# superxslam/SuperOdom

Hardware: AMD Instinct MI355X
Metric: icp_registrations_per_sec (higher is better)
Workload: dtype f64

## Files before the change

superodom_amd/csrc/kernels.hip:

```cpp
#include <hip/hip_runtime.h>
#include <hip/hip_ext.h>

#include <cstddef>
#include <cstdlib>
#include <cstring>
#include <type_traits>

#ifdef SO_LM_STAMPS
#define SO_LM_STAMP(dbg, i) do { if (dbg) (dbg)[i] = wall_clock64(); } while (0)
#endif
#include "kernels.h"
#include "plane_fit.h"

namespace soicp {

#define SO_MATCH_SUCCESS 0
#define SO_MATCH_NOT_ENOUGH 1
#define SO_MATCH_TOO_FAR 2
#define SO_MATCH_BAD_PCA 3
#define SO_MATCH_INVALID 4
#define SO_MATCH_MSE 5
#define SO_MATCH_DROPPED 254
#define SO_MATCH_PENDING 255
static_assert(SO_FIT_SUCCESS == SO_MATCH_SUCCESS && SO_FIT_BAD_PCA == SO_MATCH_BAD_PCA && SO_FIT_INVALID == SO_MATCH_INVALID && SO_FIT_MSE == SO_MATCH_MSE,
// ... 1423 lines not shown
            for (int step = 8; step >= 1; step >>= 1) r = (r + step < 16 && rowoff[r + step] <= t) ? r + step : r;
            cn[u] = rowbeg[r] + (t - rowoff[r]);
            const float4 p = mpts[cn[u]];
            ax_[u] = p.x; ay_[u] = p.y; az_[u] = p.z;
          }
        }
#pragma unroll
        for (int u = 0; u < 4; ++u)
          if (cn[u] != 0xFFFFFFFFu) loc.insert(((unsigned long long)__float_as_uint(l2_d2(qx, qy, qz, ax_[u], ay_[u], az_[u])) << 32) | cn[u]);
      }
      unsigned long long m5[5];
#pragma unroll
      for (int t = 0; t < 5; ++t) {
        m5[t] = wave_min_u64(loc.b0);
        if (loc.b0 == m5[t] && m5[t] != ~0ull) { loc.b0 = loc.b1; loc.b1 = loc.b2; loc.b2 = loc.b3; loc.b3 = loc.b4; loc.b4 = ~0ull; }
      }
      if (lane == 0) {
        const float d2_4 = __uint_as_float((uint32_t)(m5[4] >> 32));
        int stq = SO_MATCH_PENDING;
        if (m5[4] == ~0ull || (double)d2_4 > (double)mp.sq_max_dist_f) stq = SO_MATCH_TOO_FAR;
        else {
          uint32_t* o = nbr5 + (size_t)5 * i;
          __builtin_nontemporal_store((uint32_t)m5[0], o); __builtin_nontemporal_store((uint32_t)m5[1], o + 1);
          __builtin_nontemporal_store((uint32_t)m5[2], o + 2); __builtin_nontemporal_store((uint32_t)m5[3], o + 3);
          __builtin_nontemporal_store((uint32_t)m5[4], o + 4);
        }
        __builtin_nontemporal_store((uint8_t)stq, &status[i]);
      }
    }
  }
}

constexpr int kNAcc = 29;

__device__ __forceinline__ uint32_t query_of(uint32_t vb, uint32_t V, int tid, uint32_t q) { return vb * 256u + (uint32_t)tid + q * V * 256u; }

__device__ __forceinline__ bool eval_slot_active(const DevState* st, int slot) {
  return !st->reg_done && (slot == 0 || st->lm_more);
}

struct LmCtl {
  double T[7];
  int32_t lm_max, outer_iter, max_outer, pad;
};

__device__ __forceinline__ int lm_solve_finished(DevState* st, const LmCtl& ctl, const double x[7], double count, int lm_iterations,
                                                 int num_successful, int termination, double initial_cost, double x_cost, const LmSums& sums) {
  for (int i = 0; i < 7; ++i) st->T[i] = x[i];
  const int o = ctl.outer_iter;
  DevIterStats& is = st->iters[o < 16 ? o : 15];
  relative_motion(ctl.T, x, is.translation_norm, is.rotation_norm);
  is.num_surf = (int32_t)count; is.lm_iterations = lm_iterations; is.num_successful = num_successful;
  is.termination = termination; is.initial_cost = initial_cost; is.final_cost = x_cost;
  for (int h = 0; h < 7; ++h) is.reject_hist[h] = (int32_t)sums.hist[h];
  for (int h = 0; h < 9; ++h) is.obs_hist[h] = (int32_t)sums.hist[7 + h];
  for (int i = 0; i < 7; ++i) is.pose_after[i] = x[i];
  st->outer_iter = o + 1;
  st->n_iterations = o + 1;
  if (num_successful == 1 || o + 1 >= ctl.max_outer) {
    st->reg_done = 1;
    for (int i = 0; i < 7; ++i) st->T_final[i] = x[i];
    st->done_count = st->done_count + 1u;
    return 1;
  }
  return 0;
}

__device__ __forceinline__ int lm_control_regs(int slot, DevState* st, LmState& S, const LmSums& sums, const LmCtl& ctl, bool persist,
                                               int* reg_done_out = nullptr) {
  if (reg_done_out) *reg_done_out = 0;
  int more;
  double unused_pose[7];
  double* next_pose = persist ? unused_pose : st->eval_pose;
  if (slot == 0) more = lm_begin(S, ctl.T, sums, ctl.lm_max, next_pose);
#ifdef SO_LM_STAMPS
  else more = lm_feed(S, sums, next_pose, slot == 1 ? st->dbg : nullptr);
#else
  else more = lm_feed(S, sums, next_pose);
#endif
  if (!persist || !more) st->lm_more = more;
  if (more) return 1;
  const int rd = lm_solve_finished(st, ctl, S.x, S.count, S.lm_iterations, S.num_successful, S.termination, S.initial_cost, S.x_cost, sums);
  if (rd) {
    if (reg_done_out) *reg_done_out = 1;
    const bool have = S.count > 0;
    for (int i = 0; i < 36; ++i) st->JtJ[i] = have ? S.H[i] : 0.0;
    for (int i = 0; i < 6; ++i) st->Jtr[i] = have ? S.g[i] : 0.0;
  }
  return 0;
}

typedef unsigned int u4v __attribute__((ext_vector_type(4)));
__device__ __forceinline__ void store16_sc1(u4v* p, u4v v) { asm volatile("global_store_dwordx4 %0, %1, off sc1" ::"v"(p), "v"(v) : "memory"); }
__device__ __forceinline__ u4v load16_sc1(const u4v* p) {
  u4v v;
  asm volatile("global_load_dwordx4 %0, %1, off sc1\n\ts_waitcnt vmcnt(0)" : "=v"(v) : "v"(p) : "memory");
  return v;
}

__device__ __forceinline__ void store16_sys(u4v* p, u4v v) { asm volatile("global_store_dwordx4 %0, %1, off sc0 sc1" ::"v"(p), "v"(v) : "memory"); }
__device__ __forceinline__ u4v load16_sys(const u4v* p) {
  u4v v;
  asm volatile("global_load_dwordx4 %0, %1, off sc0 sc1\n\ts_waitcnt vmcnt(0)" : "=v"(v) : "v"(p) : "memory");
  return v;
}

#define SO_LM_INLINE __forceinline__
__device__ SO_LM_INLINE int lm_control(int slot, DevState* st, LmState& S_lds, const LmSums& sums_lds, const LmCtl& ctl, bool persist = false,
                                       u4v* hand = nullptr, unsigned long long want = 0, double* pose_out = nullptr, int* reg_done_out = nullptr) {
  LmState S;
#pragma unroll
  for (int i = 0; i < 7; ++i) { S.x[i] = S_lds.x[i]; S.cand[i] = S_lds.cand[i]; }
#pragma unroll
  for (int i = 0; i < 6; ++i) {
    S.g[i] = S_lds.g[i]; S.scale[i] = S_lds.scale[i]; S.diag[i] = S_lds.diag[i];
#pragma unroll
    for (int j = i; j < 6; ++j) { S.H[6 * i + j] = S_lds.H[6 * i + j]; S.H[6 * j + i] = S.H[6 * i + j]; }
  }
  S.x_cost = S_lds.x_cost; S.x_norm = S_lds.x_norm; S.inv_radius = S_lds.inv_radius; S.decrease_factor = S_lds.decrease_factor;
  S.inv_model_cost_change = S_lds.inv_model_cost_change; S.step_norm = S_lds.step_norm; S.cand_norm = S_lds.cand_norm;
  S.model_cost_change = S_lds.model_cost_change; S.initial_cost = S_lds.initial_cost; S.count = S_lds.count;
  S.iter = S_lds.iter; S.max_iter = S_lds.max_iter; S.reuse_diagonal = S_lds.reuse_diagonal; S.invalid_steps = S_lds.invalid_steps;
  S.num_successful = S_lds.num_successful; S.termination = S_lds.termination; S.done = S_lds.done; S.lm_iterations = S_lds.lm_iterations;
  const int more_ = lm_control_regs(slot, st, S, sums_lds, ctl, persist, reg_done_out);
  if (hand) {
#pragma unroll
    for (int k = 0; k < 8; ++k) {
      const unsigned long long val = (k < 7) ? (unsigned long long)__double_as_longlong(S.cand[k < 7 ? k : 0]) : (unsigned long long)more_;
      const u4v v = {(unsigned int)val, (unsigned int)(val >> 32), (unsigned int)want, (unsigned int)(want >> 32)};
      store16_sc1(hand + k, v);
    }
#pragma unroll
    for (int k = 0; k < 7; ++k) pose_out[k] = S.cand[k];
  }
#pragma unroll
  for (int i = 0; i < 7; ++i) { S_lds.x[i] = S.x[i]; S_lds.cand[i] = S.cand[i]; }
#pragma unroll
  for (int i = 0; i < 6; ++i) {
    S_lds.g[i] = S.g[i]; S_lds.scale[i] = S.scale[i]; S_lds.diag[i] = S.diag[i];
#pragma unroll
    for (int j = i; j < 6; ++j) { S_lds.H[6 * i + j] = S.H[6 * i + j]; S_lds.H[6 * j + i] = S.H[6 * i + j]; }
  }
  S_lds.x_cost = S.x_cost; S_lds.x_norm = S.x_norm; S_lds.inv_radius = S.inv_radius; S_lds.decrease_factor = S.decrease_factor;
  S_lds.inv_model_cost_change = S.inv_model_cost_change; S_lds.step_norm = S.step_norm; S_lds.cand_norm = S.cand_norm;
  S_lds.model_cost_change = S.model_cost_change; S_lds.initial_cost = S.initial_cost; S_lds.count = S.count;
  S_lds.iter = S.iter; S_lds.max_iter = S.max_iter; S_lds.reuse_diagonal = S.reuse_diagonal; S_lds.invalid_steps = S.invalid_steps;
  S_lds.num_successful = S.num_successful; S_lds.termination = S.termination; S_lds.done = S.done; S_lds.lm_iterations = S.lm_iterations;
#ifdef SO_LM_STAMPS
  if (slot == 1) st->dbg[7] = wall_clock64();
#endif
  return more_;
}

__device__ __forceinline__ int lm_control_wave(int slot, DevState* st, LmState& S, const LmSums& sums, const LmCtl& ctl, double* gather ,
                                               u4v* hand, unsigned long long want, double* pose_out, int* reg_done_out, int lane,
                                               unsigned long long* dbg = nullptr) {
  const bool is_mat = lane < 36, is_vec = lane >= 36 && lane < 42;
  const int li = is_mat ? lane / 6 : 0, lj = is_mat ? lane - 6 * li : (is_vec ? lane - 36 : 0);
  const int la = li < lj ? li : lj, lb = li < lj ? lj : li;
  const int tri = 6 * la - (la * (la - 1)) / 2 + (lb - la);
  const bool is_diag = is_mat && li == lj;
  double x[7], cand[7];
  double x_cost, x_norm, inv_radius, decrease_factor, mcc_state, initial_cost, count, inv_mcc, step_norm, cand_norm;
  int iter, max_iter, reuse_diagonal, invalid_steps, num_successful, termination, done, lm_iterations;
  double Hl = 0, gl = 0, diag_l = 0, sa = 1.0, sb = 1.0;
  int more = 0;
  bool propose = false;
  if (slot == 0) {
#pragma unroll
    for (int i = 0; i < 7; ++i) { x[i] = ctl.T[i]; cand[i] = x[i]; }
    iter = 0; max_iter = ctl.lm_max; reuse_diagonal = 0; invalid_steps = 0; num_successful = 0; termination = 0; done = 0; lm_iterations = 0;
    inv_radius = LmConst::kInitialInvRadius; decrease_factor = 2.0; mcc_state = 0; inv_mcc = 0; step_norm = 0; cand_norm = 0;
    count = sums.count; x_cost = sums.cost; initial_cost = x_cost; x_norm = 0;
    if (is_mat) Hl = sums.JtJ[tri];
    if (is_vec) gl = sums.Jtr[lj];
    if (!(count > 0)) { termination = 4; done = 1; }
    else {
      const double sc = 1.0 / (1.0 + sqrt(Hl));
      if (is_diag) S.scale[li] = sc;
      __builtin_amdgcn_fence(__ATOMIC_ACQ_REL, "wavefront");
      sa = S.scale[is_vec ? lj : la]; sb = S.scale[lb];
      double n2 = 0;
#pragma unroll
      for (int i = 0; i < 7; ++i) n2 = SO_FMA(x[i], x[i], n2);
      x_norm = sqrt(n2);
      propose = true;
    }
  } else {
#pragma unroll
    for (int i = 0; i < 7; ++i) { x[i] = S.x[i]; cand[i] = S.cand[i]; }
    x_cost = S.x_cost; x_norm = S.x_norm; inv_radius = S.inv_radius; decrease_factor = S.decrease_factor; mcc_state = S.model_cost_change;
    initial_cost = S.initial_cost; count = S.count; inv_mcc = S.inv_model_cost_change; step_norm = S.step_norm; cand_norm = S.cand_norm;
    iter = S.iter; max_iter = S.max_iter; reuse_diagonal = S.reuse_diagonal; invalid_steps = S.invalid_steps; num_successful = S.num_successful;
    termination = S.termination; done = S.done; lm_iterations = S.lm_iterations;
    if (is_mat) { Hl = S.H[lane]; sa = S.scale[la]; sb = S.scale[lb]; }
    if (is_vec) { gl = S.g[lj]; sa = S.scale[lj]; }
    if (is_diag) diag_l = S.diag[li];
    if (!done) {
      SO_LM_STAMP(dbg, 0);
      const double cand_cost = sums.cost;
      if (step_norm <= LmConst::kParameterTolerance * (x_norm + LmConst::kParameterTolerance)) { termination = 2; done = 1; }
      else {
        const double cost_change = x_cost - cand_cost;
        if (fabs(cost_change) <= LmConst::kFunctionTolerance * x_cost) { termination = 1; done = 1; }
        else {
          const double rel = cost_change * inv_mcc;
          SO_LM_STAMP(dbg, 1);
          if (rel > LmConst::kMinRelativeDecrease) {
#pragma unroll
            for (int i = 0; i < 7; ++i) x[i] = cand[i];
            x_norm = cand_norm; x_cost = cand_cost;
            if (is_mat) Hl = sums.JtJ[tri];
            if (is_vec) gl = sums.Jtr[lj];
            num_successful++;
            const double u = 2.0 * rel - 1.0;
            double f = 1.0 - u * u * u;
            if (f < 1.0 / 3.0) f = 1.0 / 3.0;
            inv_radius = inv_radius * f;
            if (inv_radius < LmConst::kMinInvRadius) inv_radius = LmConst::kMinInvRadius;
            decrease_factor = 2.0; reuse_diagonal = 0;
            if (iter >= max_iter) { termination = 0; done = 1; }
            else propose = true;
          } else {
            inv_radius = inv_radius * decrease_factor; decrease_factor *= 2.0; reuse_diagonal = 1;
            propose = true;
          }
          SO_LM_STAMP(dbg, 2);
        }
      }
    }
  }
  if (propose && reuse_diagonal == 0) {
    const double xi = lane == 36 ? x[0] : (lane == 37 ? x[1] : x[2]);
    const bool big = lane >= 36 && lane < 39 && fabs(gl) > 1e-6 && fabs(xi) < 1e5;
    if (__ballot(big) == 0ull) {
      if (is_vec) gather[48 + lj] = gl;
      __builtin_amdgcn_fence(__ATOMIC_ACQ_REL, "wavefront");
      double gu[6];
#pragma unroll
      for (int i = 0; i < 6; ++i) gu[i] = gather[48 + i];
      if (lm_gradient_max_norm(x, gu) <= LmConst::kGradientTolerance) { termination = 3; done = 1; propose = false; }
    }
  }
  double scale_u[6];
#pragma unroll
  for (int i = 0; i < 6; ++i) scale_u[i] = 1.0;
  if (propose) {
#pragma unroll
    for (int i = 0; i < 6; ++i) scale_u[i] = S.scale[i];
  }
  while (propose) {
    if (iter >= max_iter) { termination = 0; done = 1; break; }
    if (inv_radius >= LmConst::kMaxInvRadius) { termination = 5; done = 1; break; }
    iter++; lm_iterations = iter;
    if (!reuse_diagonal) {
      double v = Hl * sa * sa;
      v = v < LmConst::kMinLmDiagonal ? LmConst::kMinLmDiagonal : v;
      diag_l = v > LmConst::kMaxLmDiagonal ? LmConst::kMaxLmDiagonal : v;
    }
    const double Hs = Hl * sa * sb;
    const double damp = diag_l * inv_radius;
    const double Al = is_diag ? Hs + damp : Hs;
    if (is_mat) gather[lane] = Al;
    if (is_diag) gather[42 + li] = Hs;
    if (is_vec) gather[36 + lj] = gl * sa;
    __builtin_amdgcn_fence(__ATOMIC_ACQ_REL, "wavefront");
    double A[36], gs[6], y[6], step[6];
#pragma unroll
    for (int i = 0; i < 6; ++i) {
#pragma unroll
      for (int j = 0; j <= i; ++j) A[6 * i + j] = gather[6 * i + j];
      gs[i] = gather[36 + i];
    }
    SO_LM_STAMP(dbg, 3);
    const bool ok = lm_chol6(A, gs, y);
    SO_LM_STAMP(dbg, 4);
    reuse_diagonal = 1;
    double mcc = 0;
    if (ok) {
      double sHs = 0, sg = 0;
#pragma unroll
      for (int i = 0; i < 6; ++i) { step[i] = -y[i]; sg = SO_FMA(step[i], gs[i], sg); }
#pragma unroll
      for (int i = 0; i < 6; ++i) {
        double r = 0;
#pragma unroll
        for (int j = i + 1; j < 6; ++j) r = SO_FMA(gather[6 * i + j], step[j], r);
        sHs = SO_FMA(step[i], SO_FMA(gather[42 + i], step[i], 2.0 * r), sHs);
      }
      mcc = SO_FMA(-0.5, sHs, -sg);
    }
    __builtin_amdgcn_fence(__ATOMIC_ACQ_REL, "wavefront");
    if (!ok || !(mcc > 0.0)) {
      if (++invalid_steps >= LmConst::kMaxConsecutiveInvalidSteps) { termination = 5; done = 1; break; }
      inv_radius *= 2.0;
      continue;
    }
    SO_LM_STAMP(dbg, 5);
    invalid_steps = 0;
    mcc_state = mcc;
    double delta[6];
#pragma unroll
    for (int i = 0; i < 6; ++i) delta[i] = step[i] * scale_u[i];
    pose_plus(x, delta, cand);
    SO_LM_STAMP(dbg, 6);
    more = 1;
    break;
  }
  {
    double hv = cand[0];
    hv = lane == 1 ? cand[1] : hv; hv = lane == 2 ? cand[2] : hv; hv = lane == 3 ? cand[3] : hv;
    hv = lane == 4 ? cand[4] : hv; hv = lane == 5 ? cand[5] : hv; hv = lane == 6 ? cand[6] : hv;
    const unsigned long long val = lane == 7 ? (unsigned long long)more : (unsigned long long)__double_as_longlong(hv);
    if (lane < 8) {
      const u4v v = {(unsigned int)val, (unsigned int)(val >> 32), (unsigned int)want, (unsigned int)(want >> 32)};
      store16_sc1(hand + lane, v);
    }
    if (lane < 7) pose_out[lane] = hv;
  }
  if (more) {
    inv_mcc = 1.0 / mcc_state;
    double sn = 0, n2 = 0;
#pragma unroll
    for (int i = 0; i < 7; ++i) sn = SO_FMA(x[i] - cand[i], x[i] - cand[i], sn);
#pragma unroll
    for (int i = 0; i < 7; ++i) n2 = SO_FMA(cand[i], cand[i], n2);
    step_norm = sqrt(sn); cand_norm = sqrt(n2);
  }
  if (is_mat) S.H[lane] = Hl;
  if (is_vec) S.g[lj] = gl;
  if (is_diag) S.diag[li] = diag_l;
  if (slot == 0 && termination == 4 && lane < 6) S.scale[lane] = 1.0;
  if (lane == 0) {
#pragma unroll
    for (int i = 0; i < 7; ++i) { S.x[i] = x[i]; S.cand[i] = cand[i]; }
    S.x_cost = x_cost; S.x_norm = x_norm; S.inv_radius = inv_radius; S.decrease_factor = decrease_factor; S.model_cost_change = mcc_state;
    S.initial_cost = initial_cost; S.count = count; S.inv_model_cost_change = inv_mcc; S.step_norm = step_norm; S.cand_norm = cand_norm;
    S.iter = iter; S.max_iter = max_iter; S.reuse_diagonal = reuse_diagonal; S.invalid_steps = invalid_steps; S.num_successful = num_successful;
    S.termination = termination; S.done = done; S.lm_iterations = lm_iterations;
  }
#ifdef SO_LM_STAMPS
  if (slot == 1 && lane == 0) st->dbg[7] = wall_clock64();
#endif
  if (!more) {
    int rd = 0;
    if (lane == 0) {
      st->lm_more = 0;
      rd = lm_solve_finished(st, ctl, x, count, lm_iterations, num_successful, termination, initial_cost, x_cost, sums);
      *reg_done_out = rd;
    }
    rd = __builtin_amdgcn_readfirstlane(rd);
    if (rd) {
      const bool have = count > 0;
      if (is_mat) st->JtJ[lane] = have ? Hl : 0.0;
      if (is_vec) st->Jtr[lj] = have ? gl : 0.0;
    }
  } else if (lane == 0) *reg_done_out = 0;
  return more;
}

__device__ __forceinline__ void load_ctl(LmCtl& ctl, const DevState* st, int tid, int first) {
  const int k = tid - first;
  if (k >= 0 && k < 7) ctl.T[k] = st->T[k];
  else if (k == 7) ctl.lm_max = st->lm_max;
  else if (k == 8) ctl.outer_iter = st->outer_iter;
  else if (k == 9) ctl.max_outer = st->max_outer;
}

__device__ __forceinline__ void publish_state(const DevState* st, const EvalParams& ep, int outer, int tid, int nthreads) {
  publish_state_to(ep.hring[outer & 1], st, ep.seq_base | (unsigned long long)(outer + 1), tid, nthreads);
}
__device__ __forceinline__ void publish_state_to(DevState* dst, const DevState* st, unsigned long long seq, int tid, int nthreads) {
  if (!dst) return;
  __threadfence_block();
  __syncthreads();
  const unsigned long long* src = reinterpret_cast<const unsigned long long*>(st);
  unsigned long long* out = reinterpret_cast<unsigned long long*>(dst);
  constexpr int kWords = (int)(offsetof(DevState, seq) / 8);
  for (int i = tid; i < kWords; i += nthreads) out[i] = src[i];
  __threadfence_system();
  __syncthreads();
  if (tid == 0) __hip_atomic_store(&dst->seq, seq, __ATOMIC_RELEASE, __HIP_MEMORY_SCOPE_SYSTEM);
}

__device__ __forceinline__ void copy_words(double* dst, const double* src, int n_doubles, int tid, int nthreads) {
  for (int i = tid; i < n_doubles; i += nthreads) dst[i] = src[i];
}
static_assert(sizeof(LmState) % 8 == 0 && sizeof(LmSums) % 8 == 0, "controller state must be double-aligned");

constexpr int kPartStride = SO_SOLVE_BLOCKS;
static_assert(kEvalBlocks <= kPartStride && kFitBlocksMax <= kPartStride && kNAcc <= kSumsStride, "partials table");
constexpr int kRedStride = kNAcc + 2;

template <int CTRL>
__device__ __forceinline__ double dpp_f64(double v) {
  const int lo = __builtin_amdgcn_update_dpp(0, __double2loint(v), CTRL, 0xF, 0xF, false);
  const int hi = __builtin_amdgcn_update_dpp(0, __double2hiint(v), CTRL, 0xF, 0xF, false);
  return __hiloint2double(hi, lo);
}
__device__ __forceinline__ double swap32_add(double a, double b) {
  const auto lo = __builtin_amdgcn_permlane32_swap((unsigned)__double2loint(a), (unsigned)__double2loint(b), false, false);
  const auto hi = __builtin_amdgcn_permlane32_swap((unsigned)__double2hiint(a), (unsigned)__double2hiint(b), false, false);
  return __hiloint2double((int)hi[0], (int)lo[0]) + __hiloint2double((int)hi[1], (int)lo[1]);
}
__device__ __forceinline__ double swap16_add(double a, double b) {
  const auto lo = __builtin_amdgcn_permlane16_swap((unsigned)__double2loint(a), (unsigned)__double2loint(b), false, false);
  const auto hi = __builtin_amdgcn_permlane16_swap((unsigned)__double2hiint(a), (unsigned)__double2hiint(b), false, false);
  return __hiloint2double((int)hi[0], (int)lo[0]) + __hiloint2double((int)hi[1], (int)lo[1]);
}
template <int CTRL>
__device__ __forceinline__ double row_stage_add(double a, double b, bool up) {
  const double keep = up ? b : a, give = up ? a : b;
  return keep + dpp_f64<CTRL>(give);
}
__device__ __forceinline__ double wave_reduce_scatter(const double (&acc)[kNAcc]) {
  static_assert(kNAcc > 16 && kNAcc <= 32, "butterfly over 32 value slots");
  const int lane = (int)(threadIdx.x & 63u);
  double u[16], w[8], x[4], y[2];
#pragma unroll
  for (int a = 0; a < 16; ++a) u[a] = swap32_add(acc[a], (a + 16 < kNAcc) ? acc[a + 16] : 0.0);
#pragma unroll
  for (int a = 0; a < 8; ++a) w[a] = swap16_add(u[a], u[a + 8]);
  const bool b3 = (lane & 8) != 0, b2 = (lane & 4) != 0, b1 = (lane & 2) != 0;
#pragma unroll
  for (int a = 0; a < 4; ++a) x[a] = row_stage_add<0x128>(w[a], w[a + 4], b3);
#pragma unroll
  for (int a = 0; a < 2; ++a) y[a] = row_stage_add<0x141>(x[a], x[a + 2], b2);
  const double z = row_stage_add<0x4E>(y[0], y[1], b1);
  return z + dpp_f64<0xB1>(z);
}
__device__ __forceinline__ double wg_reduce(const double (&acc)[kNAcc], double (*part)[32], int tid) {
  const double t = wave_reduce_scatter(acc);
  const int lane = tid & 63, wave = tid >> 6;
  if (!(lane & 1) && (lane >> 1) < kNAcc) part[wave][lane >> 1] = t;
  __syncthreads();
  double tot = 0;
  if (tid < kNAcc) tot = ((part[0][tid] + part[1][tid]) + part[2][tid]) + part[3][tid];
  return tot;
}

__device__ __forceinline__ double reduce_records(double (*red)[kRedStride], double (*part)[32], int tid) {
  const int a = tid & 31, cch = tid >> 5;
  if (a < kNAcc) {
    double s = 0;
#pragma unroll 8
    for (int r = 0; r < 32; ++r) s += red[cch * 32 + r][a];
    part[cch][a] = s;
  }
  __syncthreads();
  double tot = 0;
  if (tid < kNAcc) {
#pragma unroll
    for (int cc = 0; cc < 8; ++cc) tot += part[cc][tid];
  }
  return tot;
}

struct EvalShared {
  double red[256][kRedStride];
  double part[8][32];
  double part_odd[8][32];
  LmSums sums;
  LmState S;
  LmCtl ctl;
  double pose[7];
  int more;
  int32_t lh[16];
  int32_t hpart[8][16];
  int reg_done;
  bool is_last;
  unsigned long long peer_seq;
// ... 150 lines not shown
          const float4 a = mpts[stq == SO_MATCH_PENDING ? iq[t] : 0u];
          nbq[3 * t] = a.x; nbq[3 * t + 1] = a.y; nbq[3 * t + 2] = a.z;
        }
        body(j, stq, nbq, -1);
      }
    } else
    for (uint32_t q = 0, jA; (jA = query_of(vb, V, tid, q)) < n_kept; q += 2) {
      const uint32_t jB = query_of(vb, V, tid, q + 1u);
      const bool hasB = jB < n_kept;
      const uint32_t jBs = hasB ? jB : jA;
      const int stA = corr.status[jA];
      const int stB = hasB ? (int)corr.status[jBs] : SO_MATCH_NOT_ENOUGH;
      uint32_t iA[5], iB[5];
#pragma unroll
      for (int t = 0; t < 5; ++t) { iA[t] = nbr5[(size_t)5 * jA + t]; iB[t] = nbr5[(size_t)5 * jBs + t]; }
      float nbA[15], nbB[15];
#pragma unroll
      for (int t = 0; t < 5; ++t) {
        const float4 a = mpts[stA == SO_MATCH_PENDING ? iA[t] : 0u], b = mpts[stB == SO_MATCH_PENDING ? iB[t] : 0u];
        nbA[3 * t] = a.x; nbA[3 * t + 1] = a.y; nbA[3 * t + 2] = a.z;
        nbB[3 * t] = b.x; nbB[3 * t + 1] = b.y; nbB[3 * t + 2] = b.z;
      }
      body(jA, stA, nbA, first ? 0 : -1);
      if (hasB) body(jB, stB, nbB, first ? 1 : -1);
      first = false;
    }
  } else if (PERSIST && !BATCH) {
#pragma unroll
    for (int trip = 0; trip < 2; ++trip) {
      const double c = cc->c[trip][tid];
      const double4 nd = make_double4(cc->nx[trip][tid], cc->ny[trip][tid], cc->nz[trip][tid], cc->nw[trip][tid]);
      const double px = (double)cc->px[trip][tid], py = (double)cc->py[trip][tid], pz = (double)cc->pz[trip][tid];
      if (c >= 0.0) {
        double wx, wy, wz;
        quat_rotate<double>(pose.q, px, py, pz, wx, wy, wz);
        wx += pose.t[0]; wy += pose.t[1]; wz += pose.t[2];
        tail(px, py, pz, wx, wy, wz, nd, c);
      }
    }
    for (uint32_t q = 2, j; (j = query_of(vb, V, tid, q)) < n_kept; ++q) body(j, corr.status[j], nullptr, -1);
  } else if (BATCH) {
    if (vb + 1u < vb_end) fetch2(vb + 1u, nxt);
#pragma unroll
    for (int q = 0; q < 2; ++q)
      if (cur[q].st == SO_MATCH_SUCCESS) {
        const double px = (double)cur[q].x, py = (double)cur[q].y, pz = (double)cur[q].z;
        double wx, wy, wz;
        quat_rotate<double>(pose.q, px, py, pz, wx, wy, wz);
        wx += pose.t[0]; wy += pose.t[1]; wz += pose.t[2];
        tail(px, py, pz, wx, wy, wz, cur[q].nd, cur[q].c);
      }
    for (uint32_t q = 2, j; (j = query_of(vb, V, tid, q)) < n_kept; ++q) body(j, corr.status[j], nullptr, -1);
    cur[0] = nxt[0]; cur[1] = nxt[1];
  } else {
    for (uint32_t q = 0, j; (j = query_of(vb, V, tid, q)) < n_kept; ++q) body(j, corr.status[j], nullptr, -1);
  }
  if (stamp) t_loop = wall_clock64();
  mine = wg_reduce(acc, (BATCH && (trip_ & 1u)) ? sh.part_odd : part, tid);
  if (PERSIST) {
    static_assert(SO_SOLVE_BLOCKS == 256, "record table: 8 groups of 32 workgroups");
    static_assert(kNAcc <= kRecordChunksMax, "record table");
    if (FIT) __builtin_amdgcn_s_waitcnt(0x0F70);
    if (tid < kNAcc) {
      const unsigned long long b = (unsigned long long)__double_as_longlong(mine);
      const unsigned int extra = (FIT && tid < 16 && (!BATCH || vb + 1u == vb_end)) ? (unsigned int)lh[tid] : 0u;
      const u4v v = {(unsigned int)b, (unsigned int)(b >> 32), tag, extra};
      const uint32_t w = vb;
      store16_sc1(rec + ((w & 31u) * 8u + (w >> 5)) * kNAcc + tid, v);
    }
  }
  }
  if (PERSIST) {
    if (stamp) t_red = wall_clock64();
    if (!is_ctl) return kPassNotLast;
    constexpr int kPoll = 8 * kNAcc;
    const bool poller = tid < kPoll;
    const int g = poller ? tid / kNAcc : 0, a = poller ? tid - g * kNAcc : 0;
    const u4v* base = rec + (poller ? tid : 0);
    if (!BATCH) {
    u4v r[32];
    const unsigned long long t0 = wall_clock64();
    bool ok;
    for (;;) {
#pragma unroll
      for (int i = 0; i < 32; ++i)
        asm volatile("global_load_dwordx4 %0, %1, off sc1" : "=v"(r[i]) : "v"(base + (size_t)i * kPoll) : "memory");
      asm volatile("s_waitcnt vmcnt(0)"
                   : "+v"(r[0]), "+v"(r[1]), "+v"(r[2]), "+v"(r[3]), "+v"(r[4]), "+v"(r[5]), "+v"(r[6]), "+v"(r[7]), "+v"(r[8]), "+v"(r[9]),
                     "+v"(r[10]), "+v"(r[11]), "+v"(r[12]), "+v"(r[13]), "+v"(r[14]), "+v"(r[15]), "+v"(r[16]), "+v"(r[17]), "+v"(r[18]),
                     "+v"(r[19]), "+v"(r[20]), "+v"(r[21]), "+v"(r[22]), "+v"(r[23]), "+v"(r[24]), "+v"(r[25]), "+v"(r[26]), "+v"(r[27]),
                     "+v"(r[28])
                   :: "memory");
      asm volatile("" : "+v"(r[29]), "+v"(r[30]), "+v"(r[31]) :: "memory");
      ok = true;
#pragma unroll
      for (int i = 0; i < 32; ++i) ok = ok && (r[i].z == tag || (uint32_t)(32 * g + i) >= V);
      ok = ok || !poller;
      if (abl & 8192) { ok = false; break; }
      if (__ballot(!ok) == 0ull) break;
      if (wall_clock64() - t0 > ep.timeout_ticks) break;
    }
    if (!__syncthreads_and(ok ? 1 : 0)) return kPassNotLast;
    if (stamp) t_ticket = t_loaded = wall_clock64();
    {
      double sum = 0;
      int hsum = 0;
#pragma unroll
      for (int i = 0; i < 32; ++i) {
        const bool have = (uint32_t)(32 * g + i) < V;
        sum += have ? __longlong_as_double((long long)(((unsigned long long)r[i].y << 32) | r[i].x)) : 0.0;
        if (FIT) hsum += have ? (int)r[i].w : 0;
      }
      if (poller) {
        part[g][a] = sum;
        if (FIT && a < 16) sh.hpart[g][a] = hsum;
      }
    }
    } else {
      double sum = 0;
      int hsum = 0;
      bool ok = true;
      const unsigned long long t0 = wall_clock64();
      for (int i0 = 0; i0 < 32; i0 += 8) {
        u4v r[8];
        for (;;) {
#pragma unroll
          for (int k = 0; k < 8; ++k)
            asm volatile("global_load_dwordx4 %0, %1, off sc1" : "=v"(r[k]) : "v"(base + (size_t)(i0 + k) * kPoll) : "memory");
          asm volatile("s_waitcnt vmcnt(0)" : "+v"(r[0]), "+v"(r[1]), "+v"(r[2]), "+v"(r[3]), "+v"(r[4]), "+v"(r[5]), "+v"(r[6]), "+v"(r[7]) :: "memory");
          bool good = true;
#pragma unroll
          for (int k = 0; k < 8; ++k) good = good && (r[k].z == tag || (uint32_t)(32 * g + i0 + k) >= V);
          good = good || !poller;
          if (abl & 8192) good = false;
          if (__ballot(!good) == 0ull) break;
          if ((abl & 8192) || wall_clock64() - t0 > ep.timeout_ticks) { ok = ok && good; break; }
          __builtin_amdgcn_s_sleep(32);
        }
        if (__ballot(!ok) != 0ull) break;
#pragma unroll
        for (int k = 0; k < 8; ++k) {
          const bool have = (uint32_t)(32 * g + i0 + k) < V;
          sum += have ? __longlong_as_double((long long)(((unsigned long long)r[k].y << 32) | r[k].x)) : 0.0;
          if (FIT) hsum += have ? (int)r[k].w : 0;
        }
      }
      if (!__syncthreads_and(ok ? 1 : 0)) return kPassNotLast;
      if (poller) {
        part[g][a] = sum;
        if (FIT && a < 16) sh.hpart[g][a] = hsum;
      }
    }
    __syncthreads();
    double* o = reinterpret_cast<double*>(&sh_sums);
    if (tid < kNAcc) {
      double tot = 0;
#pragma unroll
      for (int cc8 = 0; cc8 < 8; ++cc8) tot += part[cc8][tid];
      o[tid] = tot;
    } else if (FIT && tid >= 32 && tid < 48) {
      int h = 0;
#pragma unroll
      for (int cc8 = 0; cc8 < 8; ++cc8) h += sh.hpart[cc8][tid - 32];
      o[kNAcc + (tid - 32)] = (double)h;
    }
    __syncthreads();
    if (PEER && ep.peer_world > 1) {
      const int nx = FIT ? (kNAcc + 16) : kNAcc;
      const unsigned int xtag = (unsigned int)(sh.peer_seq + 1ull);
      const int par = (int)(xtag & 1u);
      if (tid < nx) {
        const unsigned long long b = (unsigned long long)__double_as_longlong(o[tid]);
        const u4v v = {(unsigned int)b, (unsigned int)(b >> 32), xtag, (unsigned int)ep.peer_rank};
        for (int p = 0; p < ep.peer_world; ++p)
          store16_sys(reinterpret_cast<u4v*>(ep.peer_inbox[p]) + (size_t)(par * kPeerMaxWorld + ep.peer_rank) * kPeerChunks + tid, v);
      }
      const u4v* own = reinterpret_cast<const u4v*>(ep.peer_inbox[ep.peer_rank]) + (size_t)par * kPeerMaxWorld * kPeerChunks;
      const int total = nx * ep.peer_world;
      const int c0 = tid, c1 = tid + 256;
      const bool h0 = c0 < total, h1 = c1 < total;
      const int s0 = h0 ? c0 / nx : 0, a0 = h0 ? c0 - s0 * nx : 0, s1 = h1 ? c1 / nx : 0, a1 = h1 ? c1 - s1 * nx : 0;
      bool d0 = !h0, d1 = !h1;
      unsigned long long v0 = 0, v1 = 0;
      const unsigned long long tp = wall_clock64();
      bool okx = true;
      for (;;) {
        if (!d0) { const u4v v = load16_sys(own + (size_t)s0 * kPeerChunks + a0); if (v.z == xtag) { d0 = true; v0 = ((unsigned long long)v.y << 32) | v.x; } }
        if (!d1) { const u4v v = load16_sys(own + (size_t)s1 * kPeerChunks + a1); if (v.z == xtag) { d1 = true; v1 = ((unsigned long long)v.y << 32) | v.x; } }
        if (__syncthreads_and((d0 && d1) ? 1 : 0)) break;
        if (__syncthreads_or((wall_clock64() - tp > ep.timeout_ticks) ? 1 : 0)) { okx = false; break; }
      }
      if (!__syncthreads_and(okx ? 1 : 0)) return kPassNotLast;
      double (*xs)[48] = reinterpret_cast<double (*)[48]>(&red[0][0]);
      if (h0) xs[s0][a0] = __longlong_as_double((long long)v0);
      if (h1) xs[s1][a1] = __longlong_as_double((long long)v1);
      __syncthreads();
      if (tid < nx) {
        double tot = 0;
        for (int r = 0; r < ep.peer_world; ++r) tot += xs[r][tid];
        o[tid] = tot;
      }
      if (tid == 0) sh.peer_seq = (unsigned long long)xtag;
      __syncthreads();
    }
    if (stamp) t_sums = wall_clock64();
    if (tid < 64) {
#ifdef SO_LM_STAMPS
      const int more_ = lm_control_wave(slot, st, sh_S, sh_sums, sh_ctl, &sh.part_odd[0][0], hand, want, sh.pose, &sh.reg_done, tid, (slot == 1 && tid == 0) ? st->dbg : nullptr);
#else
      const int more_ = lm_control_wave(slot, st, sh_S, sh_sums, sh_ctl, &sh.part_odd[0][0], hand, want, sh.pose, &sh.reg_done, tid);
#endif
      if (tid == 0) sh_more = more_;
    }
    __syncthreads();
    unsigned long long t_ctl = 0;
    if (stamp) t_ctl = wall_clock64();
    if (!sh_more) {
      hist[tid] = 0; hist[256 + tid] = 0;
      if (PEER && ep.peer_world > 1 && tid == 0) st->peer_seq = sh.peer_seq;
      if (tid < (int)(sizeof(LmState) / 8))
        __hip_atomic_store(reinterpret_cast<double*>(&st->S) + tid, reinterpret_cast<const double*>(&sh_S)[tid], __ATOMIC_RELAXED, __HIP_MEMORY_SCOPE_AGENT);
      if (!BATCH && ep.chain_next && sh.reg_done && tid == 0) {
        double tf[7], nx[7];
        for (int i = 0; i < 7; ++i) tf[i] = sh_S.x[i];
        pose_compose(tf, ep.chain_delta, nx);
        for (int i = 0; i < 7; ++i) st->T_chain[i] = nx[i];
      }
      if (!ep.defer_publish || sh.reg_done) publish_state(st, ep, sh_ctl.outer_iter, tid, 256);
    }
    if (stamp && tid == 0 && (FIT || slot == 1)) {
      t_lm = wall_clock64();
      unsigned long long* d = st->dbg + (FIT ? 0 : 8);
      d[0] = t_loop - t_begin; d[1] = t_red - t_loop; d[2] = t_ticket - t_red; d[3] = t_loaded - t_ticket; d[4] = t_sums - t_loaded;
      d[5] = t_lm - t_sums; d[6] = t_lm - t_begin; d[7] = t_ctl - t_sums;
    }
    return sh_more ? kPassMore : kPassDone;
  }
  if (tid < kNAcc)
    __hip_atomic_store(&partials[(size_t)tid * kPartStride + blockIdx.x], mine, __ATOMIC_RELAXED, __HIP_MEMORY_SCOPE_AGENT);
  if (FIT && tid >= 32 && tid < 48 && lh[tid - 32])
    __hip_atomic_fetch_add(&hist[(blockIdx.x % kHistReplicas) * kHistStride + (tid - 32)], lh[tid - 32], __ATOMIC_RELAXED, __HIP_MEMORY_SCOPE_AGENT);
  asm volatile("s_waitcnt vmcnt(0)" ::: "memory");
  __syncthreads();
  if (stamp) t_red = wall_clock64();
  if (tid == 0) __hip_atomic_fetch_add(&ticket[(blockIdx.x & (kArriveCounters - 1)) * kArriveStrideWords], 1u, __ATOMIC_RELAXED, __HIP_MEMORY_SCOPE_AGENT);
  if (blockIdx.x != 0) return kPassNotLast;
  if (tid < 64) {
    const uint32_t lanes = kArriveCounters;
    const uint32_t expect = (tid < (int)lanes) ? (gridDim.x + lanes - 1u - (uint32_t)tid) / lanes : 0u;
    const unsigned long long t0 = wall_clock64();
    bool ok = false;
    for (;;) {
      uint32_t v = 0;
      if (tid < (int)lanes) v = __hip_atomic_load(&ticket[tid * kArriveStrideWords], __ATOMIC_RELAXED, __HIP_MEMORY_SCOPE_AGENT);
      if (__ballot(v != expect) == 0ull) { ok = true; break; }
      if (wall_clock64() - t0 > ep.timeout_ticks) break;
    }
    if (tid < (int)lanes) __hip_atomic_store(&ticket[tid * kArriveStrideWords], 0u, __ATOMIC_RELAXED, __HIP_MEMORY_SCOPE_AGENT);
    if (tid == 0) is_last = ok;
  }
  __syncthreads();
  if (!is_last) return kPassNotLast;
  if (stamp) t_ticket = wall_clock64();
  {
    constexpr int kRec = (SO_SOLVE_BLOCKS + 255) / 256;
    double r[kRec][kNAcc];
    bool have[kRec];
#pragma unroll
    for (int q = 0; q < kRec; ++q) {
      have[q] = (uint32_t)(tid + 256 * q) < gridDim.x;
      const double* rec = partials + (have[q] ? tid + 256 * q : 0);
#pragma unroll
      for (int a = 0; a < kNAcc; ++a)
        asm volatile("global_load_dwordx2 %0, %1, off sc1" : "=v"(r[q][a]) : "v"(rec + a * kPartStride) : "memory");
    }
    if (fuse_lm) {
      if (!keep_state && tid < (int)(sizeof(LmState) / 8))
        reinterpret_cast<double*>(&sh_S)[tid] = __hip_atomic_load(reinterpret_cast<const double*>(&st->S) + tid, __ATOMIC_RELAXED, __HIP_MEMORY_SCOPE_AGENT);
      load_ctl(sh_ctl, st, tid, 128);
    }
#pragma unroll
    for (int q = 0; q < kRec; ++q)
      asm volatile("s_waitcnt vmcnt(0)"
                   : "+v"(r[q][0]), "+v"(r[q][1]), "+v"(r[q][2]), "+v"(r[q][3]), "+v"(r[q][4]), "+v"(r[q][5]), "+v"(r[q][6]), "+v"(r[q][7]),
                     "+v"(r[q][8]), "+v"(r[q][9]), "+v"(r[q][10]), "+v"(r[q][11]), "+v"(r[q][12]), "+v"(r[q][13]), "+v"(r[q][14]),
                     "+v"(r[q][15]), "+v"(r[q][16]), "+v"(r[q][17]), "+v"(r[q][18]), "+v"(r[q][19]), "+v"(r[q][20]), "+v"(r[q][21]),
                     "+v"(r[q][22]), "+v"(r[q][23]), "+v"(r[q][24]), "+v"(r[q][25]), "+v"(r[q][26]), "+v"(r[q][27]), "+v"(r[q][28])
                   :: "memory");
#pragma unroll
    for (int a = 0; a < kNAcc; ++a) {
      double v = have[0] ? r[0][a] : 0.0;
#pragma unroll
      for (int q = 1; q < kRec; ++q) v += have[q] ? r[q][a] : 0.0;
      red[tid][a] = v;
    }
  }
  __syncthreads();
  if (stamp) t_loaded = wall_clock64();
  const double total = reduce_records(red, part, tid);
  double* o = reinterpret_cast<double*>(&sh_sums);
  if (tid < kNAcc) {
    o[tid] = total;
  } else if (tid >= 32 && tid < 48) {
    int h = 0;
#pragma unroll
    for (int r = 0; r < kHistReplicas; ++r)
      h += __hip_atomic_load(&hist[r * kHistStride + (tid - 32)], __ATOMIC_RELAXED, __HIP_MEMORY_SCOPE_AGENT);
    o[kNAcc + (tid - 32)] = (double)h;
  }
  __syncthreads();
  copy_words(reinterpret_cast<double*>(out), o, (int)(sizeof(LmSums) / 8), tid, 256);
  if (stamp) t_sums = wall_clock64();
  if (!fuse_lm) return kPassSums;
  if (tid == 0) sh_more = (abl & 32) ? 1 : lm_control(slot, st, sh_S, sh_sums, sh_ctl);
  __syncthreads();
  unsigned long long t_ctl = 0;
  if (stamp) t_ctl = wall_clock64();
  if (!sh_more) { hist[tid] = 0; hist[256 + tid] = 0; }
  if ((!keep_state || !sh_more) && tid < (int)(sizeof(LmState) / 8))
    __hip_atomic_store(reinterpret_cast<double*>(&st->S) + tid, reinterpret_cast<const double*>(&sh_S)[tid], __ATOMIC_RELAXED, __HIP_MEMORY_SCOPE_AGENT);
  if (!sh_more) publish_state(st, ep, sh_ctl.outer_iter, tid, 256);
  if (stamp && tid == 0 && (FIT || slot == 1)) {
    t_lm = wall_clock64();
    unsigned long long* d = st->dbg + (FIT ? 0 : 8);
    d[0] = t_loop - t_begin; d[1] = t_red - t_loop; d[2] = t_ticket - t_red; d[3] = t_loaded - t_ticket; d[4] = t_sums - t_loaded;
    d[5] = t_lm - t_sums; d[6] = t_lm - t_begin; d[7] = t_ctl - t_sums;
  }
  return sh_more ? kPassMore : kPassDone;
}

static_assert(sizeof(LmState) / 8 <= 256, "controller state is moved one word per thread");
template <bool FIT, bool PROF>
__global__ __launch_bounds__(256, SO_SOLVE_BLOCKS / 256) void eval_kernel(int slot, int fuse_lm, const float* __restrict__ spx,
                                                   const float* __restrict__ spy, const float* __restrict__ spz,
                                                   CorrBuffers corr, DevState* __restrict__ st, EvalParams ep,
                                                   double* __restrict__ partials, uint32_t* __restrict__ ticket,
                                                   int32_t* __restrict__ hist, LmSums* __restrict__ out,
                                                   const float4* __restrict__ mpts, const uint32_t* __restrict__ nbr5,
                                                   MatchParams mp) {
  __shared__ EvalShared sh;
  if (!eval_slot_active(st, slot)) return;
  const Pose pose = pose_from_array(slot == 0 ? st->T : st->eval_pose);
  (void)eval_pass<FIT, false, PROF>(slot, fuse_lm, pose, spx, spy, spz, corr, st, ep, partials, ticket, hist, out, mpts, nbr5, mp, sh);
}

template <bool PROF, bool BATCH, bool PEER = false>
__global__ __launch_bounds__(256, BATCH ? 2 : 1) void solve_kernel(int lm_max, const float* __restrict__ spx, const float* __restrict__ spy,
                                                    const float* __restrict__ spz, CorrBuffers corr, DevState* __restrict__ st,
                                                    EvalParams ep, double* __restrict__ partials, uint32_t* __restrict__ ticket,
                                                    int32_t* __restrict__ hist, LmSums* __restrict__ out,
                                                    const float4* __restrict__ mpts, const uint32_t* __restrict__ nbr5,
                                                    MatchParams mp, BatchView bv) {
  __shared__ EvalShared sh;
  __shared__ CorrCache cache;
  WgSpan span{0, 0, 0, false};
  if (BATCH) {
    const uint32_t G = bv.wg_per_hyp, hi = blockIdx.x / G, sub = blockIdx.x - hi * G;
    const size_t h = bv.active[hi];
    st += h; corr.nd += h * bv.bs; corr.coeff += h * bv.bs; corr.status += h * bv.bs; nbr5 += h * 5 * bv.bs;
    partials += h * bv.partial_stride; ticket += h * bv.sync_stride; hist += h * (kHistReplicas * kHistStride);
    span.V = bv.v_grid;
    span.vb0 = (uint32_t)(((unsigned long long)sub * bv.v_grid) / G);
    span.vb1 = (uint32_t)(((unsigned long long)(sub + 1u) * bv.v_grid) / G);
    span.ctl = sub == 0;
// ... 304 lines not shown
```

Before: 7131.

## Fold partial-sum reduction into LM control wave and drop a block barrier

Result: faster. 7234 (median of 6 runs) (+1.5%).

```diff
diff --git a/superodom_amd/csrc/kernels.hip b/superodom_amd/csrc/kernels.hip
--- a/superodom_amd/csrc/kernels.hip
+++ b/superodom_amd/csrc/kernels.hip
@@ -1599,14 +1599,27 @@
   return more_;
 }
 
-__device__ __forceinline__ int lm_control_wave(int slot, DevState* st, LmState& S, const LmSums& sums, const LmCtl& ctl, double* gather ,
+template <bool SINGLE>
+__device__ __forceinline__ int lm_control_wave(int slot, DevState* st, LmState& S, LmSums& sums, const LmCtl& ctl, double* gather ,
                                                u4v* hand, unsigned long long want, double* pose_out, int* reg_done_out, int lane,
+                                               const double (*part)[32] = nullptr, const int32_t (*hpart)[16] = nullptr,
                                                unsigned long long* dbg = nullptr) {
   const bool is_mat = lane < 36, is_vec = lane >= 36 && lane < 42;
   const int li = is_mat ? lane / 6 : 0, lj = is_mat ? lane - 6 * li : (is_vec ? lane - 36 : 0);
   const int la = li < lj ? li : lj, lb = li < lj ? lj : li;
   const int tri = 6 * la - (la * (la - 1)) / 2 + (lb - la);
   const bool is_diag = is_mat && li == lj;
+  double s_cost, s_count, s_el;
+  if (SINGLE && part) {
+    const int e = is_mat ? 8 + tri : 2 + lj;
+    double c0 = 0, c1 = 0, t = 0;
+#pragma unroll
+    for (int g = 0; g < 8; ++g) { c0 += part[g][0]; c1 += part[g][1]; t += part[g][e]; }
+    s_cost = c0; s_count = c1; s_el = t;
+  } else {
+    s_cost = sums.cost; s_count = sums.count;
+    s_el = is_mat ? sums.JtJ[tri] : sums.Jtr[lj];
+  }
   double x[7], cand[7];
   double x_cost, x_norm, inv_radius, decrease_factor, mcc_state, initial_cost, count, inv_mcc, step_norm, cand_norm;
   int iter, max_iter, reuse_diagonal, invalid_steps, num_successful, termination, done, lm_iterations;
@@ -1618,9 +1631,9 @@
     for (int i = 0; i < 7; ++i) { x[i] = ctl.T[i]; cand[i] = x[i]; }
     iter = 0; max_iter = ctl.lm_max; reuse_diagonal = 0; invalid_steps = 0; num_successful = 0; termination = 0; done = 0; lm_iterations = 0;
     inv_radius = LmConst::kInitialInvRadius; decrease_factor = 2.0; mcc_state = 0; inv_mcc = 0; step_norm = 0; cand_norm = 0;
-    count = sums.count; x_cost = sums.cost; initial_cost = x_cost; x_norm = 0;
-    if (is_mat) Hl = sums.JtJ[tri];
-    if (is_vec) gl = sums.Jtr[lj];
+    count = s_count; x_cost = s_cost; initial_cost = x_cost; x_norm = 0;
+    if (is_mat) Hl = s_el;
+    if (is_vec) gl = s_el;
     if (!(count > 0)) { termination = 4; done = 1; }
     else {
       const double sc = 1.0 / (1.0 + sqrt(Hl));
@@ -1645,7 +1658,7 @@
     if (is_diag) diag_l = S.diag[li];
     if (!done) {
       SO_LM_STAMP(dbg, 0);
-      const double cand_cost = sums.cost;
+      const double cand_cost = s_cost;
       if (step_norm <= LmConst::kParameterTolerance * (x_norm + LmConst::kParameterTolerance)) { termination = 2; done = 1; }
       else {
         const double cost_change = x_cost - cand_cost;
@@ -1657,8 +1670,8 @@
 #pragma unroll
             for (int i = 0; i < 7; ++i) x[i] = cand[i];
             x_norm = cand_norm; x_cost = cand_cost;
-            if (is_mat) Hl = sums.JtJ[tri];
-            if (is_vec) gl = sums.Jtr[lj];
+            if (is_mat) Hl = s_el;
+            if (is_vec) gl = s_el;
             num_successful++;
             const double u = 2.0 * rel - 1.0;
             double f = 1.0 - u * u * u;
@@ -1712,19 +1725,24 @@
     if (is_diag) gather[42 + li] = Hs;
     if (is_vec) gather[36 + lj] = gl * sa;
     __builtin_amdgcn_fence(__ATOMIC_ACQ_REL, "wavefront");
-    double A[36], gs[6], y[6], step[6];
+    double A[36], gs[6], y[6], step[6], Hu[36], Hd[6];
 #pragma unroll
     for (int i = 0; i < 6; ++i) {
 #pragma unroll
       for (int j = 0; j <= i; ++j) A[6 * i + j] = gather[6 * i + j];
       gs[i] = gather[36 + i];
+      if (SINGLE) {
+        Hd[i] = gather[42 + i];
+#pragma unroll
+        for (int j = i + 1; j < 6; ++j) Hu[6 * i + j] = gather[6 * i + j];
+      }
     }
     SO_LM_STAMP(dbg, 3);
     const bool ok = lm_chol6(A, gs, y);
     SO_LM_STAMP(dbg, 4);
     reuse_diagonal = 1;
     double mcc = 0;
-    if (ok) {
+    if (SINGLE || ok) {
       double sHs = 0, sg = 0;
 #pragma unroll
       for (int i = 0; i < 6; ++i) { step[i] = -y[i]; sg = SO_FMA(step[i], gs[i], sg); }
@@ -1732,13 +1750,14 @@
       for (int i = 0; i < 6; ++i) {
         double r = 0;
 #pragma unroll
-        for (int j = i + 1; j < 6; ++j) r = SO_FMA(gather[6 * i + j], step[j], r);
-        sHs = SO_FMA(step[i], SO_FMA(gather[42 + i], step[i], 2.0 * r), sHs);
+        for (int j = i + 1; j < 6; ++j) r = SO_FMA(SINGLE ? Hu[6 * i + j] : gather[6 * i + j], step[j], r);
+        sHs = SO_FMA(step[i], SO_FMA(SINGLE ? Hd[i] : gather[42 + i], step[i], 2.0 * r), sHs);
       }
       mcc = SO_FMA(-0.5, sHs, -sg);
     }
-    __builtin_amdgcn_fence(__ATOMIC_ACQ_REL, "wavefront");
+    if (!SINGLE) __builtin_amdgcn_fence(__ATOMIC_ACQ_REL, "wavefront");
     if (!ok || !(mcc > 0.0)) {
+      if (SINGLE) __builtin_amdgcn_fence(__ATOMIC_ACQ_REL, "wavefront");
       if (++invalid_steps >= LmConst::kMaxConsecutiveInvalidSteps) { termination = 5; done = 1; break; }
       inv_radius *= 2.0;
       continue;
@@ -1764,6 +1783,15 @@
       store16_sc1(hand + lane, v);
     }
     if (lane < 7) pose_out[lane] = hv;
+  }
+  if (SINGLE && hpart) {
+    if (lane < 16) {
+      int h = 0;
+#pragma unroll
+      for (int g = 0; g < 8; ++g) h += hpart[g][lane];
+      sums.hist[lane] = (double)h;
+    }
+    __builtin_amdgcn_fence(__ATOMIC_ACQ_REL, "wavefront");
   }
   if (more) {
     inv_mcc = 1.0 / mcc_state;
@@ -2220,19 +2248,22 @@
       }
     }
     __syncthreads();
+    const bool lane_combine = !BATCH && !(PEER && ep.peer_world > 1);
     double* o = reinterpret_cast<double*>(&sh_sums);
-    if (tid < kNAcc) {
-      double tot = 0;
-#pragma unroll
-      for (int cc8 = 0; cc8 < 8; ++cc8) tot += part[cc8][tid];
-      o[tid] = tot;
-    } else if (FIT && tid >= 32 && tid < 48) {
-      int h = 0;
-#pragma unroll
-      for (int cc8 = 0; cc8 < 8; ++cc8) h += sh.hpart[cc8][tid - 32];
-      o[kNAcc + (tid - 32)] = (double)h;
-    }
-    __syncthreads();
+    if (!lane_combine) {
+      if (tid < kNAcc) {
+        double tot = 0;
+#pragma unroll
+        for (int cc8 = 0; cc8 < 8; ++cc8) tot += part[cc8][tid];
+        o[tid] = tot;
+      } else if (FIT && tid >= 32 && tid < 48) {
+        int h = 0;
+#pragma unroll
+        for (int cc8 = 0; cc8 < 8; ++cc8) h += sh.hpart[cc8][tid - 32];
+        o[kNAcc + (tid - 32)] = (double)h;
+      }
+      __syncthreads();
+    }
     if (PEER && ep.peer_world > 1) {
       const int nx = FIT ? (kNAcc + 16) : kNAcc;
       const unsigned int xtag = (unsigned int)(sh.peer_seq + 1ull);
@@ -2274,10 +2305,16 @@
     if (stamp) t_sums = wall_clock64();
     if (tid < 64) {
 #ifdef SO_LM_STAMPS
-      const int more_ = lm_control_wave(slot, st, sh_S, sh_sums, sh_ctl, &sh.part_odd[0][0], hand, want, sh.pose, &sh.reg_done, tid, (slot == 1 && tid == 0) ? st->dbg : nullptr);
+      unsigned long long* dbg = (slot == 1 && tid == 0) ? st->dbg : nullptr;
 #else
-      const int more_ = lm_control_wave(slot, st, sh_S, sh_sums, sh_ctl, &sh.part_odd[0][0], hand, want, sh.pose, &sh.reg_done, tid);
+      unsigned long long* dbg = nullptr;
 #endif
+      int more_;
+      if constexpr (BATCH)
+        more_ = lm_control_wave<false>(slot, st, sh_S, sh_sums, sh_ctl, &sh.part_odd[0][0], hand, want, sh.pose, &sh.reg_done, tid, nullptr, nullptr, dbg);
+      else
+        more_ = lm_control_wave<true>(slot, st, sh_S, sh_sums, sh_ctl, &sh.part_odd[0][0], hand, want, sh.pose, &sh.reg_done, tid,
+                                      lane_combine ? part : nullptr, (lane_combine && FIT) ? sh.hpart : nullptr, dbg);
       if (tid == 0) sh_more = more_;
     }
     __syncthreads();
```
